# QWERTY6191/projected-lmc

Measured on AMD Instinct MI355X. Metric: MLL+grad iters/sec, n=8192 16-task LMC, higher is better.
Workload: dtype f32; 1 GPU; C3: ProjectedGPModel+ProjectedLMCmll exact training step (PLMC_fast), n=8192 d=8 p=16 q=8 Matern-5/2 fp32; latents sharded q/N per GPU; n_points=8192, n_dim=8, n_tasks=16, n_latents=8, parallelism=latent-shard x1

## Files before the change

### include/plmc.h

```cpp
#ifndef PLMC_H
#define PLMC_H

#include <stddef.h>
#include <stdint.h>

#ifdef __cplusplus
extern "C" {
#endif

enum { PLMC_RBF = 0, PLMC_MATERN12 = 1, PLMC_MATERN32 = 2, PLMC_MATERN52 = 3, PLMC_SPLINE = 4 };

int         plmc_version(void);
int         plmc_block(void);
int64_t     plmc_pad(int64_t n);
int         plmc_max_dim(void);
const char *plmc_last_error(void);
int64_t     plmc_vd_blocks_for(int64_t n_pad, int64_t lda, int elem_bytes);
int64_t     plmc_vd_blocks(int64_t n_pad, int64_t lda);
int64_t     plmc_vd_blocks_keep(int64_t n_pad, int64_t lda);
int64_t     plmc_split_scales_offset(int64_t n_pad, int64_t lda);
int64_t     plmc_grad_scratch_bytes_for(int64_t n_pad, int q, int elem_bytes);
int64_t     plmc_grad_scratch_bytes(int64_t n_pad, int q);
int64_t     plmc_grad_partials_bytes(int64_t n_pad, int q);

// ... 35 lines not shown
int plmc_potrs_aug_f64(double *A, int64_t n_pad, int64_t lda, int naug, int64_t wcol0, int64_t strideA, double *Vd, int q, void *stream);
int plmc_potrs_aug_kept_f32(float *A, int64_t n_pad, int64_t lda, int naug, int64_t wcol0, int64_t strideA, float *Vd, int q,
                            const float *eig_lo, void *stream);
int plmc_potrs_aug_kept_f64(double *A, int64_t n_pad, int64_t lda, int naug, int64_t wcol0, int64_t strideA, double *Vd, int q,
                            const double *eig_lo, void *stream);

int plmc_extract_col_f32(const float *A, int64_t n_pad, int64_t lda, int64_t strideA, int c,
                         float *z, double *quad, int q, void *stream);
int plmc_extract_col_f64(const double *A, int64_t n_pad, int64_t lda, int64_t strideA, int c,
                         double *z, double *quad, int q, void *stream);

int plmc_wt_matvec_f32(const float *W, int64_t n_pad, int64_t ldw, int64_t strideW, const float *z,
                       float *alpha, int q, void *stream);
int plmc_wt_matvec_f64(const double *W, int64_t n_pad, int64_t ldw, int64_t strideW, const double *z,
                       double *alpha, int q, void *stream);

int plmc_trmm_ut_f32(const float *A, int64_t n_pad, int64_t lda, int64_t strideA, int n, const float *Z, int ns, int64_t ldz,
                     int64_t strideZ, const float *shift, float *Y, int64_t ldy, int64_t strideY, int q, void *stream);
int plmc_trmm_ut_f64(const double *A, int64_t n_pad, int64_t lda, int64_t strideA, int n, const double *Z, int ns, int64_t ldz,
                     int64_t strideZ, const double *shift, double *Y, int64_t ldy, int64_t strideY, int q, void *stream);

int plmc_gemm_tn_f32(int mode, int M, int N, int K, const float *A, int64_t lda, int64_t strideA, const float *B,
                     int64_t ldb, int64_t strideB, float *C, int64_t ldc, int64_t strideC, int batch, void *stream);
int plmc_gemm_tn_f64(int mode, int M, int N, int K, const double *A, int64_t lda, int64_t strideA, const double *B,
                     int64_t ldb, int64_t strideB, double *C, int64_t ldc, int64_t strideC, int batch, void *stream);
#define PLMC_TRI_A_LOWER 1
#define PLMC_TRI_B_LOWER 2
#define PLMC_TRI_A_UPPER 4
#define PLMC_TRI_C_LOWER 8
#define PLMC_TRI_C_ZERO 16
// ... 520 lines not shown
```

### projected-lmc_amd/csrc/api.hip

```cpp
#include <stdlib.h>
#include <mutex>
#include <vector>

#include "api_common.hpp"
#include "../../include/plmc.h"

namespace plmc {
char *err_buf() {
  static thread_local char buf[256] = {0};
  return buf;
}

static const char *kProfNames[PK_COUNT] = {"k_assemble", "k_write_rhs", "k_assemble_cross", "k_diag",   "k_panel",
                                           "k_trail",    "k_wdiag",     "k_trtri_row",      "k_extract_col",
                                           "k_wt_matvec", "k_kinv_grad", "k_reduce_grad", "k_kernel_vjp",
                                           "sweep_total", "k_trail_row", "k_trail_head", "k_gpanel", "k_split_w", "k_posterior_moments", "k_trmm_ut",
                                           "k_input_grad", "k_posterior_dx", "k_cross_matvec", "k_cross_matvec_dx"};
struct ProfRec { int id; hipEvent_t a, b; double flops, bytes; };
static unsigned g_prof_mask = 0;
static std::vector<ProfRec> g_recs;
static std::vector<hipEvent_t> g_free;

static hipEvent_t get_event() {
  if (!g_free.empty()) { hipEvent_t e = g_free.back(); g_free.pop_back(); return e; }
// ... 9 lines not shown
static Knobs g_knobs;
static bool g_knobs_loaded = false;
static void load_knobs() {
  const char *h = getenv("PLMC_HALF_TILES"), *g = getenv("PLMC_GRP");
  g_knobs.half_tiles = h ? (atoi(h) == 1 ? 1e30 : (double)atoi(h)) : 640.0;
  g_knobs.grp = g ? atoi(g) : 0;
  g_knobs.serial = getenv("PLMC_SERIAL") && atoi(getenv("PLMC_SERIAL")) != 0;
  g_knobs.bulk_lds = getenv("PLMC_BULK_LDS") ? atoi(getenv("PLMC_BULK_LDS")) : -1;
  g_knobs.split = getenv("PLMC_SPLIT") ? atoi(getenv("PLMC_SPLIT")) : 2;
  if (g_knobs.split != 0 && g_knobs.split != 3) g_knobs.split = 2;
  g_knobs.bulk_streams = getenv("PLMC_BULK_STREAMS") ? atoi(getenv("PLMC_BULK_STREAMS")) : 2;
  g_knobs.chain = getenv("PLMC_CHAIN") ? atoi(getenv("PLMC_CHAIN")) : 1;
  g_knobs.chain_nw = getenv("PLMC_CHAIN_NW") ? atoi(getenv("PLMC_CHAIN_NW")) : 0;
  g_knobs.tail_pair = getenv("PLMC_TAIL_PAIR") ? atoi(getenv("PLMC_TAIL_PAIR")) : 1;
  g_knobs.chain_edge = getenv("PLMC_CHAIN_EDGE") ? atoi(getenv("PLMC_CHAIN_EDGE")) : 0;
  g_knobs_loaded = true;
}
const Knobs &knobs() {
  if (!g_knobs_loaded) {
    std::lock_guard<std::recursive_mutex> lk(g_api_mutex);
    if (!g_knobs_loaded) load_knobs();
  }
  return g_knobs;
}

constexpr int SWEEP_CTX = 2;
struct SweepCtx {
  hipStream_t caller = nullptr;
  bool used = false;
  unsigned long long stamp = 0;
// ... 177 lines not shown
```

### projected-lmc_amd/csrc/api_common.hpp

```cpp
#pragma once
#include <hip/hip_runtime.h>
#include <stdint.h>
#include <stdio.h>
#include <string.h>
#include <type_traits>

#include "gemm_core.hpp"
#include "covariance.hpp"

namespace plmc {

constexpr int MAX_DIM = 32;
constexpr int MAX_COMP = 4;
constexpr int SM_MAX_MIX = 8;
constexpr int SM_MAX_DIM = 8;
constexpr int PER_MAX_DIM = 8;
constexpr int RQ_MAX_DIM = 16;
constexpr int LPER_MAX_DIM = 8;
constexpr int DOT_MAX_DIM = 16;
constexpr int DOT_MAX_POWER = 8;
constexpr int SUM_MAX_DIM = 8;
constexpr int FAM_PUBLIC_BASE = 16;
enum { F_PER = 5, F_RQ = 6, F_LPER = 7 };

// ... 27 lines not shown
  long idx_;
  hipStream_t st_;
};

struct Knobs {
  double half_tiles;
  int grp;
  bool serial;
  int bulk_lds;
  int split;
  int bulk_streams;
  int chain;
  int chain_edge;
  int tail_pair;
  int chain_nw;
};
const Knobs &knobs();

enum CovFamily { COV_PLAIN, COV_ADD, COV_SM, COV_PER, COV_RQ, COV_LPER, COV_SUM, COV_DOT };

constexpr int EVERY_D = 1 << 30, NEVER = 1 << 30;
struct FamilyTraits {
  int max_dim;
  const char *dim_text;
  int max_count;
  const char *count_text;
  bool count_first;
  bool needs_second, needs_third;
  bool rows_per_comp;
  int max_dc;
// ... 142 lines not shown
```

### projected-lmc_amd/csrc/potrf.hip

```cpp
#include <stdlib.h>
#include "api_common.hpp"
#include "covariance.hpp"
#include "diag_block.hpp"
#include "bf3_engine.hpp"
#include "chain_engine.hpp"
#include "vd_layout.hpp"
#include "../../include/plmc.h"

namespace plmc {

template <typename T> constexpr int CHAIN_BURST = sizeof(T) == 8 ? 4 : 8;

template <typename T> struct ColMap {
  int u0, nU, Taug, w0, nW;
  int64_t n_pad;
  T *W;
  int64_t ldw, strideW;
};

template <typename T, int NT, bool BURSTED = false>
__global__ __launch_bounds__(NTHREADS, TILE_MIN_WAVES<T>) void k_panel(T *A, int64_t lda, int64_t strideA, int r, ColMap<T> cm,
                                                     const T *__restrict__ Vd, int64_t strideV) {
  __builtin_amdgcn_s_setprio(3);
  __shared__ __align__(16) T smem[tile_smem_elems<T>()];
// ... 596 lines not shown
    for (int u = 0; u < U; ++u)
#pragma unroll
      for (int e = 0; e < EPV; ++e) s[e] += (double)v[u][e] * (double)zz[u];
  }
#pragma unroll
  for (int e = 0; e < EPV; ++e) red[rg][cl + e] = s[e];
  __syncthreads();
  if (threadIdx.x < CW) {
    double t = 0.0;
#pragma unroll
    for (int g = 0; g < NRG; ++g) t += red[g][threadIdx.x];
    alpha[(int64_t)lat * n_pad + colw + threadIdx.x] = (T)t;
  }
}

template <typename T>
__global__ __launch_bounds__(WTMV_NT) void k_w_diag(const T *__restrict__ W, int64_t n_pad, int64_t ldw, int64_t strideW,
                                                    T *__restrict__ kd) {
  using vec_t = typename Traits<T>::vec_t;
  constexpr int EPV = Traits<T>::EPV;
  constexpr int LPR = 128 / EPV;
  constexpr int NRG = WTMV_NT / LPR;
  __shared__ double red[NRG][NB];
  const int lat = blockIdx.y;
  const int cl = (threadIdx.x % LPR) * EPV, rg = threadIdx.x / LPR;
  const int64_t col0 = (int64_t)blockIdx.x * NB;
  const T *Wl = W + (int64_t)lat * strideW + col0 + cl;
  double s[EPV];
#pragma unroll
  for (int e = 0; e < EPV; ++e) s[e] = 0.0;
// ... 8 lines not shown
    for (int u = 0; u < 4; ++u)
      if (l + u * NRG < n_pad) {
#pragma unroll
        for (int e = 0; e < EPV; ++e) s[e] += (double)v[u][e] * (double)v[u][e];
      }
  }
#pragma unroll
  for (int e = 0; e < EPV; ++e) red[rg][cl + e] = s[e];
  __syncthreads();
  if (threadIdx.x < NB) {
    double t = 0.0;
#pragma unroll
    for (int g = 0; g < NRG; ++g) t += red[g][threadIdx.x];
    kd[(int64_t)lat * n_pad + col0 + threadIdx.x] = (T)t;
  }
}

template <typename T, class S>
struct Sweep {
  static constexpr bool bf3 = !std::is_void<S>::value;
  static_assert(!bf3 || sizeof(T) == 4, "split schemes stand in for fp32 products");
  static constexpr double nb = NB, nb3 = nb * nb * nb, esz = sizeof(T);

  T *A;
  int64_t n_pad, lda, strideA, naug_pad, wcol0;
  int q, m, Taug;
  bool with_inverse, keep;
  const float *eig_lo = nullptr;
  double *logdet = nullptr;
  int *info = nullptr;
  T *Vd, *Wg, *Vg2[2], *Ph, *Pbulk;
  unsigned short *Pl[2], *Praw, *VgP2[2], *Wk, *Uk;
  unsigned short *Pl4 = nullptr;
  float *scl;
  int64_t strideV, pl_lat, sc_lat, uk_step;
  int64_t slot_step = 0;
  bool pair = false;
  T *WA;
  const Knobs &kn;
  double hthr;
  unsigned bulk_lds;
  int grp, ng, chain_pool;
  hipStream_t st, C = nullptr, H = nullptr;
  hipEvent_t e_entry = nullptr, e_v = nullptr, e_gh = nullptr, e_p = nullptr, e_hd = nullptr, e_tail = nullptr, e_doneC = nullptr,
             e_doneH = nullptr, e_prev = nullptr, e_sc = nullptr;

  Sweep(T *A_, int64_t n_pad_, int64_t lda_, int naug, int64_t wcol0_, int64_t strideA_, T *Vd_, int q_, bool with_inverse_, bool keep_,
        int grp_, unsigned bulk_lds_, hipStream_t st_)
      : A(A_), n_pad(n_pad_), lda(lda_), strideA(strideA_), naug_pad(plmc_pad(naug)), wcol0(wcol0_), q(q_), m((int)(n_pad_ / NB)),
        Taug((int)(plmc_pad(naug) / NB)), with_inverse(with_inverse_), keep(keep_), Vd(Vd_), kn(knobs()), hthr(kn.half_tiles),
        bulk_lds(bulk_lds_), grp(grp_), st(st_) {
    const VdLayout L(n_pad, lda, (int)sizeof(T), keep);
    strideV = L.stride();
    pl_lat = L.stride_u16();
    sc_lat = L.stride_f32();
    Wg = L.at<T>(Vd, L.wg);
    Ph = L.at<T>(Vd, L.ph);
// ... 177 lines not shown
      const int nt = cm.nU + cm.Taug + cm.nW;
      if (nt > 0)
        hipLaunchKernelGGL((k_raw_planes<S>), dim3(nt, G0(1), q), dim3(NTHREADS), 0, s, (const float *)A, lda, strideA, 0, cm, Praw, pl_lat, wcol0,
                           (const float *)scl, sc_lat);
    }
  }

  void near(int gi, hipStream_t s) {
    const int g1 = G0(gi + 1), g2 = G0(gi + 2), g3 = G0(gi + 3);
    update(g2, g3 - g2, pair_lo(gi), g1 - 1, cm_buf(g2, m - g2, Taug, 0, g1), s, PK_TRAIL, 0, 0, false, 0, true);
  }
  void far(int gi, hipStream_t s) {
    if (!(gi & 1)) return;
    const int g1 = G0(gi + 1), g3 = G0(gi + 3);
    update(g3, m - g3, pair_lo(gi), g1 - 1, cm_buf(g3, m - g3, Taug, 0, g1), s, PK_TRAIL);
  }

  bool bind_streams() {
    if (!kn.serial) bind_sweep_ctx(st, 8);
    C = kn.serial ? nullptr : side_stream();
    H = kn.serial ? nullptr : (kn.bulk_streams == 1 ? st : side_stream(1));
    hipEvent_t *const ev[] = {&e_entry, &e_v, &e_gh, &e_p, &e_hd, &e_tail, &e_doneC, &e_doneH, &e_prev};
    bool la = C && H && ng > 2;
    for (int i = 0; i < 9; ++i) la = (*ev[i] = sync_event(i)) && la;
    e_sc = sync_event(12);
    return la;
  }

  int inputs(const AssembleJob *job) {
    if (job) {
// ... 18 lines not shown
        gpanel(g0, g1 - g0, cm_buf(g1, g2 - g1, 0, 0, 0), gi & 1, st, 1);
        gpanel(g0, g1 - g0, cm_buf(g2, m - g2, Taug, 0, g0), gi & 1, st, 0);
        if (pair) {
          update(g1, g2 - g1, g0, g1 - 1, cm_buf(g2, m - g2, Taug, 0, g1), st, PK_TRAIL_HEAD, 0, 0, false, g2);
          near(gi, st);
          far(gi, st);
        } else {
          update(g1, m - g1, g0, g1 - 1, cm_buf(g1, m - g1, Taug, 0, g1), st, PK_TRAIL, g2, g2, false, g2);
        }
        update(g1, g2 - g1, g0, g1 - 1, cm_buf(g1, g2 - g1, 0, 0, 0), st, PK_TRAIL_HEAD, 0, 0, true);
      } else {
        gpanel(g0, g1 - g0, cm_buf(g1, m - g1, Taug, 0, g0), gi & 1, st, 0);
        update(g1, m - g1, g0, g1 - 1, cm_buf(g1, m - g1, Taug, 0, g1), st, PK_TRAIL);
      }
    }
    return finish(st);
  }

  int lookahead(const AssembleJob *job) {
    const bool fused = job && e_sc;
    if (fused) {
      const int rc = assemble_rows(*job, (int)sizeof(T), A, lda, strideA, q, 0, G0(1), st, G0(1));
      if (rc != 0) return rc;
      scan(st, 0, (int64_t)G0(1) * NB, 0, SCAN_PARTS / 2);
    } else {
      const int rc = inputs(job);
      if (rc != 0) return rc;
    }
    (void)hipEventRecord(e_entry, st);
    (void)hipStreamWaitEvent(C, e_entry, 0);
// ... 15 lines not shown
      (void)hipEventRecord(e_v, C);
      if (gi > 0 || bf3) (void)hipStreamWaitEvent(C, e_hd, 0);
      gpanel(g0, G, cm_buf(g1, g2 - g1, 0, 0, 0), gi & 1, C, 1);
      (void)hipEventRecord(e_gh, C);
      if (gi > 0) (void)hipStreamWaitEvent(C, e_tail, 0);
      update(g1, g2 - g1, g0, g1 - 1, cm_buf(g1, g2 - g1, 0, 0, 0), C, PK_TRAIL_HEAD, 0, 0, true);

      (void)hipStreamWaitEvent(H, e_v, 0);
      wtri_planes(gi, H);
      gpanel(g0, G, cm_buf(g2, m - g2, Taug, 0, g0), gi & 1, H, 0);
      (void)hipEventRecord(e_p, H);
      (void)hipStreamWaitEvent(H, e_gh, 0);
      if (gi > 0) (void)hipStreamWaitEvent(H, e_tail, 0);
      update(g1, g2 - g1, g0, g1 - 1, cm_buf(g2, m - g2, Taug, 0, g1), H, PK_TRAIL_HEAD, 0, 0, false, g2);
      (void)hipEventRecord(e_hd, H);

      (void)hipStreamWaitEvent(st, e_p, 0);
      (void)hipStreamWaitEvent(st, e_gh, 0);
      if (pair) {
        near(gi, st);
        (void)hipEventRecord(e_tail, st);
        far(gi, st);
      } else {
        update(g2, m - g2, g0, g1 - 1, cm_buf(g2, m - g2, Taug, 0, g1), st, PK_TRAIL);
        (void)hipEventRecord(e_tail, st);
      }
    }
    const int rc_fin = finish(C);
    (void)hipEventRecord(e_doneC, C);
    (void)hipEventRecord(e_doneH, H);
    (void)hipStreamWaitEvent(st, e_doneC, 0);
    (void)hipStreamWaitEvent(st, e_doneH, 0);
    (void)hipEventRecord(e_prev, st);
    return rc_fin;
  }
};

template <typename T, class S>
int potrf_impl(T *A, int64_t n_pad, int64_t lda, int naug, int64_t strideA, T *Vd, double *logdet, int *info,
               int with_inverse_arg, int q, const float *eig_lo, void *stream, const AssembleJob *job = nullptr) {
  PLMC_REQUIRE((with_inverse_arg & 2) == 0, "with_inverse bit 1 (K^-1 accumulated in the sweep) is gone: use plmc_kinv_grad_* behind the sweep");
  const bool with_inverse = (with_inverse_arg & 1) != 0;
  const bool keep = !std::is_void<S>::value && (with_inverse_arg & 4) != 0 && with_inverse;
  PLMC_REQUIRE(A && Vd && logdet && info, "null pointer");
  PLMC_REQUIRE(n_pad > 0 && n_pad % NB == 0 && lda % NB == 0 && lda >= n_pad, "n_pad/lda must be multiples of NB");
  const int64_t naug_pad = plmc_pad(naug);
  PLMC_REQUIRE(naug >= 0 && n_pad + naug_pad + (with_inverse ? n_pad : 0) <= lda,
               "lda too small for naug (+ the n_pad columns of the inverse factor)");
  PLMC_REQUIRE(q > 0 && aligned16(A) && aligned16(Vd), "bad q or unaligned buffer");
  const Knobs &kn = knobs();
  const int grp = (!keep && kn.grp > 0 && kn.grp < GMAX) ? kn.grp : GMAX;
  const unsigned bulk_lds = (unsigned)(kn.bulk_lds >= 0 ? kn.bulk_lds : (q == 1 ? 20000 : (q == 2 ? 16000 : 0)));
  Sweep<T, S> sw(A, n_pad, lda, naug, n_pad + naug_pad, strideA, Vd, q, with_inverse, keep, grp, bulk_lds, (hipStream_t)stream);
  sw.eig_lo = eig_lo;
  sw.logdet = logdet;
  sw.info = info;
  const double npd = (double)n_pad;
  ProfScope whole(PK_SWEEP, sw.st, q * (with_inverse ? 2.0 : 1.0) * npd * npd * npd / 3.0, 0.0);
  sw.clear();
  return sw.bind_streams() ? sw.lookahead(job) : sw.one_stream(job);
}

bool vd_w_planes(const float *Vd, int64_t n_pad, int64_t lda, const unsigned short **wk, int64_t *wk_lat_stride, const float **w_scale,
                 int64_t *w_scale_lat_stride) {
  const VdLayout L(n_pad, lda, 4, false);
  if (L.wk < 0) return false;
  *wk = L.at<const unsigned short>(Vd, L.wk);
  *wk_lat_stride = L.stride_u16();
  *w_scale = L.at<const float>(Vd, L.scl) + SC_SW;
  *w_scale_lat_stride = L.stride_f32();
  return true;
// ... 70 lines not shown
                   void *stream) {
  PLMC_REQUIRE(W && z && alpha, "null pointer");
  PLMC_REQUIRE(q > 0 && n_pad > 0 && n_pad % NB == 0 && ldw >= n_pad, "q > 0, n_pad a positive multiple of NB, ldw >= n_pad");
  PLMC_REQUIRE(aligned16(W) && ldw % Traits<T>::EPV == 0 && strideW % Traits<T>::EPV == 0, "16-byte alignment of W, ldw and strideW");
  ProfScope ps(PK_WTMV, (hipStream_t)stream, q * (double)n_pad * n_pad, q * ((double)n_pad * n_pad / 2) * sizeof(T));
  if ((int64_t)q * (n_pad / NB) < 128)
    hipLaunchKernelGGL((k_wt_matvec<T, 32>), dim3((unsigned)(n_pad / 32), q), dim3(WTMV_NT / 4), 0, (hipStream_t)stream, W, n_pad, ldw, strideW, z,
                       alpha);
  else
    hipLaunchKernelGGL((k_wt_matvec<T, NB>), dim3((unsigned)(n_pad / NB), q), dim3(WTMV_NT), 0, (hipStream_t)stream, W, n_pad, ldw, strideW, z,
                       alpha);
  return launch_status(__func__);
}

template <typename T>
int w_diag_impl(const T *W, int64_t n_pad, int64_t ldw, int64_t strideW, T *kinv_diag, int q, void *stream) {
  PLMC_REQUIRE(W && kinv_diag, "null pointer");
  PLMC_REQUIRE(q > 0 && n_pad > 0 && n_pad % NB == 0 && ldw >= n_pad, "q > 0, n_pad a positive multiple of NB, ldw >= n_pad");
  PLMC_REQUIRE(aligned16(W) && ldw % Traits<T>::EPV == 0 && strideW % Traits<T>::EPV == 0, "16-byte alignment of W, ldw and strideW");
  ProfScope ps(PK_WTMV, (hipStream_t)stream, q * (double)n_pad * n_pad, q * ((double)n_pad * n_pad / 2) * sizeof(T));
  hipLaunchKernelGGL(k_w_diag<T>, dim3((unsigned)(n_pad / NB), q), dim3(WTMV_NT), 0, (hipStream_t)stream, W, n_pad, ldw, strideW,
                     kinv_diag);
  return launch_status(__func__);
}

}

static int potrf_f32_any(float *A, int64_t n_pad, int64_t lda, int naug, int64_t strideA, float *Vd, double *logdet, int *info,
                         int with_inverse, int q, const float *eig_lo, void *stream, const plmc::AssembleJob *job = nullptr) {
  const int split = plmc::knobs().split;
// ... 65 lines not shown
                         int q, void *stream) {
  return plmc::extract_col_impl<float>(A, n_pad, lda, strideA, c, z, quad, q, stream);
}
int plmc_extract_col_f64(const double *A, int64_t n_pad, int64_t lda, int64_t strideA, int c, double *z,
                         double *quad, int q, void *stream) {
  return plmc::extract_col_impl<double>(A, n_pad, lda, strideA, c, z, quad, q, stream);
}
int plmc_wt_matvec_f32(const float *W, int64_t n_pad, int64_t ldw, int64_t strideW, const float *z, float *alpha,
                       int q, void *stream) {
  return plmc::wt_matvec_impl<float>(W, n_pad, ldw, strideW, z, alpha, q, stream);
}
int plmc_wt_matvec_f64(const double *W, int64_t n_pad, int64_t ldw, int64_t strideW, const double *z, double *alpha,
                       int q, void *stream) {
  return plmc::wt_matvec_impl<double>(W, n_pad, ldw, strideW, z, alpha, q, stream);
}
int plmc_w_diag_f32(const float *W, int64_t n_pad, int64_t ldw, int64_t strideW, float *kinv_diag, int q, void *stream) {
  return plmc::w_diag_impl<float>(W, n_pad, ldw, strideW, kinv_diag, q, stream);
}
int plmc_w_diag_f64(const double *W, int64_t n_pad, int64_t ldw, int64_t strideW, double *kinv_diag, int q, void *stream) {
  return plmc::w_diag_impl<double>(W, n_pad, ldw, strideW, kinv_diag, q, stream);
}
}
```

### projected-lmc_amd/projectedlmc/_engine.py

```python
import ctypes
import math
import os

import torch

from . import _hip
from . import settings
from .kernels import dot_power
from ._pivot import PivotCheck, deferred_pivot_checks, walk

LOG2PI = math.log(2.0 * math.pi)


class Workspace:

    def __init__(self, n, q, naug, dtype, device, with_inverse=True, keep_planes=False, ncomp=1, sm=False, per=False):
        L = _hip.lib()
        self.n, self.q, self.naug, self.dtype, self.device = n, q, naug, dtype, device
        self.ncomp = ncomp
        self.with_inverse = bool(with_inverse)
        self.keep_planes = bool(keep_planes) and self.with_inverse and dtype == torch.float32
        self.NB = L.cdll.plmc_block()
        self.n_pad = int(L.cdll.plmc_pad(n))
        self.naug_pad = int(L.cdll.plmc_pad(naug)) if naug > 0 else 0
# ... 4 lines not shown
        self.strideA = self.n_pad * self.lda
        esz = torch.empty((), dtype=dtype).element_size()
        vd_blocks = L.cdll.plmc_vd_blocks_keep(self.n_pad, self.lda) if self.keep_planes else L.cdll.plmc_vd_blocks_for(self.n_pad, self.lda, esz)
        self.Vd = torch.empty(q, int(vd_blocks), self.NB, self.NB, dtype=dtype, device=device)
        self.m = self.n_pad // self.NB
        self.A = torch.empty(q, self.n_pad, self.lda, dtype=dtype, device=device)
        self.logdet = torch.empty(q, dtype=torch.float64, device=device)
        self.quad = torch.empty(q, dtype=torch.float64, device=device)
        self.info = torch.empty(q, dtype=torch.int32, device=device)
        self.z = torch.empty(q, self.n_pad, dtype=dtype, device=device)
        self.W = self.alpha = self.partials = None
        if with_inverse:
            self.W = self.A[:, :, self.wcol0:self.wcol0 + self.n_pad]
            self.ldw, self.strideW = self.lda, self.strideA
            self.alpha = torch.empty(q, self.n_pad, dtype=dtype, device=device)
            nbytes = int(L.cdll.plmc_sm_grad_partials_bytes(self.n_pad, q, ncomp, esz) if sm
                         else L.cdll.plmc_sum_grad_partials_bytes(self.n_pad, q, ncomp, esz) if per == SUM
                         else L.cdll.plmc_lper_grad_partials_bytes(self.n_pad, q, esz) if per == LPER
                         else L.cdll.plmc_per_grad_partials_bytes(self.n_pad, q, esz) if per
                         else L.cdll.plmc_grad_partials_bytes(self.n_pad, q * ncomp))
            self.partials = torch.empty(nbytes // 8, dtype=torch.float64, device=device)


_ws_cache = {}


def _release(ws):
    pending = getattr(ws, "pending", None)
    if pending is not None:
        torch.cuda.current_stream(ws.device).wait_event(pending)
# ... 228 lines not shown
            means.record_stream(stream)
        L.call(_SM[base], dt, *head[1:], ell.shape[2], _hip.ptr(scales), _hip.ptr(means), *tail)
    elif ell.dim() == 3:
        L.call(_ADD[base], dt, *head, ell.shape[1], _hip.ptr(ell), *tail)
    else:
        L.call(base, dt, *head, _hip.ptr(ell), *tail)


def _split_grad_table(g, ell_shape, os_shape):
    ne = 1
    for s_ in ell_shape[1:]:
        ne *= s_
    return g[:, :ne].reshape(ell_shape), g[:, ne], (None if os_shape is None else g[:, ne + 1:].reshape(os_shape))


def factorize(kind, X, ell, oscale, noise, rhs, ws, Xs=None, eig_lo=True):
    L = _hip.lib()
    dt, dev = ws.dtype, ws.device
    st = _hip.stream_ptr(dev)
    k = kind_code(kind)
    q, n, d = ws.q, ws.n, X.shape[1]
    fused = os.environ.get("PLMC_FUSED_ASSEMBLE", "1") != "0"
    if not fused:
        _kernel_call(L, "plmc_assemble", dt, (k, _hip.ptr(X), n, d), ell, (_hip.ptr(oscale), _hip.ptr(noise),
                     _hip.ptr(ws.A), ws.lda, ws.strideA, q, st))
    nrhs = 0 if rhs is None else rhs.shape[1]
    if ws.naug_pad > 0:
        L.call("plmc_write_rhs", dt, _hip.ptr(rhs), nrhs, n, _hip.ptr(ws.A), ws.lda, ws.strideA, 0, ws.naug_pad, q, st)
    if Xs is not None:
        _kernel_call(L, "plmc_assemble_cross", dt, (k, _hip.ptr(X), n, _hip.ptr(Xs), Xs.shape[0], d), ell,
                     (_hip.ptr(oscale), _hip.ptr(ws.A), ws.lda, ws.strideA, ws.n_pad + nrhs, ws.n_pad, q, st))
    flags = (1 | (4 if ws.keep_planes else 0)) if ws.with_inverse else 0
    bound = _hip.ptr(noise) if eig_lo else None
    if fused:
        _kernel_call(L, "plmc_factorize_ex", dt, (k, _hip.ptr(X), n, d), ell, (_hip.ptr(oscale), _hip.ptr(noise), _hip.ptr(ws.A), ws.n_pad,
                     ws.lda, ws.naug, ws.strideA, _hip.ptr(ws.Vd), _hip.ptr(ws.logdet), _hip.ptr(ws.info), flags, q, bound, st))
    else:
        L.call("plmc_potrf_ex", dt, _hip.ptr(ws.A), ws.n_pad, ws.lda, ws.naug, ws.strideA, _hip.ptr(ws.Vd),
               _hip.ptr(ws.logdet), _hip.ptr(ws.info), flags, q, bound, st)


def factorize_checked(kind, X, ell, oscale, noise, rhs, ws, Xs=None, eig_lo=True):
    factorize(kind, X, ell, oscale, noise, rhs, ws, Xs, eig_lo)
    if not settings.check_cholesky.on():
        return 0.0
    check = PivotCheck.eager(ws)
    if not check.failed():
# ... 19 lines not shown
        if dt not in (torch.float32, torch.float64):
            raise TypeError("projectedlmc hot path supports float32 and float64 tensors")
        q, n = y.shape
        d = X.shape[1]
        _check_kernel_shape(L, ell, kind)
        G = n_components(ell, kind)
        need_grad = any(ctx.needs_input_grad[1:5]) or table is not None or x_grad
        Xc, ellc, osc, nzc, yc = (_contig(t, dt) for t in (X, ell, oscale, noise, y))
        ws = get_workspace(n, q, 1, dt, dev, need_grad, G, is_sm(ell), _per_kind(kind))
        st = _hip.stream_ptr(dev)
        grad = table if table is not None else (torch.empty(q, grad_table_width(ell, kind), dtype=torch.float64, device=dev) if need_grad else None)
        check = settings.check_cholesky.on()
        gX = torch.empty(q, n, d, dtype=torch.float64, device=dev) if x_grad else None

        def enqueue(noise_eff):
            factorize(kind, Xc, ellc, osc, noise_eff, yc.reshape(q, 1, n), ws)
            info = PivotCheck(ws) if check else None
            L.call("plmc_extract_col", dt, _hip.ptr(ws.A), ws.n_pad, ws.lda, ws.strideA, 0, _hip.ptr(ws.z),
                   _hip.ptr(ws.quad), q, st)
            if need_grad:
                L.call("plmc_wt_matvec", dt, _hip.ptr(ws.W), ws.n_pad, ws.ldw, ws.strideW, _hip.ptr(ws.z),
                       _hip.ptr(ws.alpha), q, st)
                gs = grad_stream(dev)
                gst = st
                if gs is not None:
                    gs.wait_stream(torch.cuda.current_stream(dev))
                    gst = _hip.stream_handle(gs, dev)
                    for t in (grad, Xc, ellc, osc, noise_eff, gX):
                        if t is not None:
                            t.record_stream(gs)
                Kinv = _kinv_buffer(ws) if x_grad else None
                ldk = Kinv.shape[2] if x_grad else 0
                _kernel_call(L, "plmc_kinv_grad_vd", dt, (kind_code(kind), _hip.ptr(ws.W), ws.n_pad, ws.ldw, ws.strideW,
                             _hip.ptr(ws.alpha), _hip.ptr(Xc), n, d), ellc, (_hip.ptr(osc), _hip.ptr(grad),
                             _hip.ptr(Kinv), ldk, ws.n_pad * ldk, None, _hip.ptr(ws.partials), q, _hip.ptr(noise_eff), _hip.ptr(ws.Vd), gst),
                             stream=gs)
                if x_grad:
# ... 679 lines not shown
```

### projected-lmc_amd/projectedlmc/_hip.py

```python
import ctypes
import os

import torch

_HERE = os.path.dirname(os.path.abspath(__file__))
LIB_PATH = os.environ.get("PLMC_LIB") or os.path.join(_HERE, "libplmc_hip.so")

ABI_VERSION = 4
KIND = {"rbf": 0, "matern12": 1, "matern32": 2, "matern52": 3, "spline": 4}
FAM = {"rbf": 0, "matern12": 1, "matern32": 2, "matern52": 3, "periodic": 16, "rq": 17, "locally_periodic": 18}

_c = ctypes
_P = _c.c_void_p
_I = _c.c_int
_L = _c.c_int64

_TYPED = {
    "plmc_assemble": [_I, _P, _I, _I, _P, _P, _P, _P, _L, _L, _I, _P],
    "plmc_assemble_add": [_I, _P, _I, _I, _I, _P, _P, _P, _P, _L, _L, _I, _P],
    "plmc_assemble_per": [_P, _I, _I, _P, _P, _P, _P, _P, _L, _L, _I, _P],
    "plmc_assemble_lper": [_P, _I, _I, _P, _P, _P, _P, _P, _P, _L, _L, _I, _P],
    "plmc_assemble_sum": [_P, _I, _I, _I, _P, _P, _P, _P, _P, _L, _L, _I, _P],
    "plmc_assemble_rq": [_P, _I, _I, _P, _P, _P, _P, _P, _L, _L, _I, _P],
    "plmc_assemble_dot": [_P, _I, _I, _P, _P, _I, _P, _P, _P, _L, _L, _I, _P],
# ... 9 lines not shown
    "plmc_assemble_cross_sm": [_P, _I, _P, _I, _I, _I, _P, _P, _P, _P, _L, _L, _L, _L, _I, _P],
    "plmc_potrf": [_P, _L, _L, _I, _L, _P, _P, _P, _I, _I, _P],
    "plmc_potrf_ex": [_P, _L, _L, _I, _L, _P, _P, _P, _I, _I, _P, _P],
    "plmc_factorize_ex": [_I, _P, _I, _I, _P, _P, _P, _P, _L, _L, _I, _L, _P, _P, _P, _I, _I, _P, _P],
    "plmc_factorize_add_ex": [_I, _P, _I, _I, _I, _P, _P, _P, _P, _L, _L, _I, _L, _P, _P, _P, _I, _I, _P, _P],
    "plmc_factorize_per_ex": [_P, _I, _I, _P, _P, _P, _P, _P, _L, _L, _I, _L, _P, _P, _P, _I, _I, _P, _P],
    "plmc_factorize_lper_ex": [_P, _I, _I, _P, _P, _P, _P, _P, _P, _L, _L, _I, _L, _P, _P, _P, _I, _I, _P, _P],
    "plmc_factorize_sum_ex": [_P, _I, _I, _I, _P, _P, _P, _P, _P, _L, _L, _I, _L, _P, _P, _P, _I, _I, _P, _P],
    "plmc_factorize_rq_ex": [_P, _I, _I, _P, _P, _P, _P, _P, _L, _L, _I, _L, _P, _P, _P, _I, _I, _P, _P],
    "plmc_factorize_dot_ex": [_P, _I, _I, _P, _P, _I, _P, _P, _P, _L, _L, _I, _L, _P, _P, _P, _I, _I, _P, _P],
    "plmc_factorize_sm_ex": [_P, _I, _I, _I, _P, _P, _P, _P, _P, _L, _L, _I, _L, _P, _P, _P, _I, _I, _P, _P],
    "plmc_potrs_aug": [_P, _L, _L, _I, _L, _L, _P, _I, _P],
    "plmc_potrs_aug_kept": [_P, _L, _L, _I, _L, _L, _P, _I, _P, _P],
    "plmc_extract_col": [_P, _L, _L, _L, _I, _P, _P, _I, _P],
    "plmc_wt_matvec": [_P, _L, _L, _L, _P, _P, _I, _P],
    "plmc_w_diag": [_P, _L, _L, _L, _P, _I, _P],
    "plmc_trmm_ut": [_P, _L, _L, _L, _I, _P, _I, _L, _L, _P, _P, _L, _L, _I, _P],
    "plmc_gemm_tn": [_I, _I, _I, _I, _P, _L, _L, _P, _L, _L, _P, _L, _L, _I, _P],
    "plmc_gemm_tn_tri": [_I, _I, _I, _I, _I, _P, _L, _L, _P, _L, _L, _P, _L, _L, _I, _P],
    "plmc_kinv_grad": [_I, _P, _L, _L, _L, _P, _P, _I, _I, _P, _P, _P, _P, _L, _L, _P, _P, _I, _P],
    "plmc_kinv_grad_ex": [_I, _P, _L, _L, _L, _P, _P, _I, _I, _P, _P, _P, _P, _L, _L, _P, _P, _I, _P, _P],
    "plmc_kinv_grad_vd": [_I, _P, _L, _L, _L, _P, _P, _I, _I, _P, _P, _P, _P, _L, _L, _P, _P, _I, _P, _P, _P],
    "plmc_kinv_grad_add_vd": [_I, _P, _L, _L, _L, _P, _P, _I, _I, _I, _P, _P, _P, _P, _L, _L, _P, _P, _I, _P, _P, _P],
    "plmc_kinv_grad_per_vd": [_P, _L, _L, _L, _P, _P, _I, _I, _P, _P, _P, _P, _P, _L, _L, _P, _P, _I, _P, _P, _P],
    "plmc_kinv_grad_lper_vd": [_P, _L, _L, _L, _P, _P, _I, _I, _P, _P, _P, _P, _P, _P, _L, _L, _P, _P, _I, _P, _P, _P],
    "plmc_kinv_grad_sum_vd": [_P, _L, _L, _L, _P, _P, _I, _I, _I, _P, _P, _P, _P, _P, _L, _L, _P, _P, _I, _P, _P, _P],
    "plmc_kinv_grad_rq_vd": [_P, _L, _L, _L, _P, _P, _I, _I, _P, _P, _P, _P, _P, _L, _L, _P, _P, _I, _P, _P, _P],
    "plmc_kinv_grad_dot_vd": [_P, _L, _L, _L, _P, _P, _I, _I, _P, _P, _I, _P, _P, _P, _L, _L, _P, _P, _I, _P, _P, _P],
    "plmc_kinv_grad_sm_vd": [_P, _L, _L, _L, _P, _P, _I, _I, _I, _P, _P, _P, _P, _P, _L, _L, _P, _P, _I, _P, _P, _P],
    "plmc_loo_grad": [_I, _P, _L, _L, _L, _L, _P, _P, _I, _I, _P, _P, _P, _P, _I, _P],
# ... 45 lines not shown
    "plmc_kernel_vjp": [_I, _P, _I, _P, _I, _I, _P, _P, _P, _L, _L, _P, _P, _P, _I, _P],
    "plmc_kernel_vjp_add": [_I, _P, _I, _P, _I, _I, _I, _P, _P, _P, _L, _L, _P, _P, _P, _I, _P],
    "plmc_qr_small": [_P, _I, _I, _L, _P, _L, _P, _L, _P],
    "plmc_comm_allreduce_sum": [_P, _L, _P],
    "plmc_posterior_moments": [_P, _L, _L, _L, _I, _P, _P, _I, _P],
    "plmc_mix_posterior": [_P, _P, _P, _I, _I, _I, _c.c_double, _P, _P, _P],
}
_PLAIN = {
    "plmc_version": ([], _I),
    "plmc_block": ([], _I),
    "plmc_pad": ([_L], _L),
    "plmc_vd_blocks": ([_L, _L], _L),
    "plmc_vd_blocks_for": ([_L, _L, _I], _L),
    "plmc_vd_blocks_keep": ([_L, _L], _L),
    "plmc_split_scales_offset": ([_L, _L], _L),
    "plmc_max_dim": ([], _I),
    "plmc_max_components": ([], _I),
    "plmc_sm_max_mixtures": ([], _I),
    "plmc_sm_max_dim": ([], _I),
    "plmc_sm_grad_partials_bytes": ([_L, _I, _I, _I], _L),
    "plmc_per_max_dim": ([], _I),
    "plmc_per_grad_partials_bytes": ([_L, _I, _I], _L),
    "plmc_lper_max_dim": ([], _I),
    "plmc_lper_grad_partials_bytes": ([_L, _I, _I], _L),
    "plmc_sum_max_components": ([], _I),
    "plmc_sum_max_dim": ([], _I),
    "plmc_sum_grad_partials_bytes": ([_L, _I, _I, _I], _L),
    "plmc_rq_max_dim": ([], _I),
    "plmc_dot_max_dim": ([], _I),
    "plmc_dot_max_power": ([], _I),
# ... 158 lines not shown
```

Measured before the change: 60.77 iters/sec.

## Overlap W^T z matvec with Cholesky sweep via per-group partial accumulation

Splits the alpha = W^T z matvec into row-range partial sums that are launched on the head stream as each group of the inverse factor finishes, accumulating into a float64 buffer. A final kernel adds the last group's rows, writes alpha, and also extracts z and the quadratic term, replacing the separate extract_col and wt_matvec launches. The goal is to hide the matvec inside the factorization sweep and remove a full serial pass over W after it. The cost is extra launches, an fp64 accumulator buffer, and reliance on thread-local arming state shared between the Python and C layers.

Result: no change. 61.30 iters/sec, median of 6 (+0.9%).

```diff
diff --git a/include/plmc.h b/include/plmc.h
--- a/include/plmc.h
+++ b/include/plmc.h
@@ -73,6 +73,10 @@
                        float *alpha, int q, void *stream);
 int plmc_wt_matvec_f64(const double *W, int64_t n_pad, int64_t ldw, int64_t strideW, const double *z,
                        double *alpha, int q, void *stream);
+
+int plmc_alpha_partials_arm_f32(float *z, double *quad, float *alpha, double *acc, int c, void *stream);
+int plmc_alpha_partials_arm_f64(double *z, double *quad, double *alpha, double *acc, int c, void *stream);
+int plmc_alpha_partials_ranges(int64_t n_pad, int grp, int64_t *r0r1, int cap);
 
 int plmc_trmm_ut_f32(const float *A, int64_t n_pad, int64_t lda, int64_t strideA, int n, const float *Z, int ns, int64_t ldz,
                      int64_t strideZ, const float *shift, float *Y, int64_t ldy, int64_t strideY, int q, void *stream);
diff --git a/projected-lmc_amd/csrc/api.hip b/projected-lmc_amd/csrc/api.hip
--- a/projected-lmc_amd/csrc/api.hip
+++ b/projected-lmc_amd/csrc/api.hip
@@ -47,6 +47,7 @@
   g_knobs.chain_nw = getenv("PLMC_CHAIN_NW") ? atoi(getenv("PLMC_CHAIN_NW")) : 0;
   g_knobs.tail_pair = getenv("PLMC_TAIL_PAIR") ? atoi(getenv("PLMC_TAIL_PAIR")) : 1;
   g_knobs.chain_edge = getenv("PLMC_CHAIN_EDGE") ? atoi(getenv("PLMC_CHAIN_EDGE")) : 0;
+  g_knobs.alpha_partials = getenv("PLMC_ALPHA_PARTIALS") ? atoi(getenv("PLMC_ALPHA_PARTIALS")) : 1;
   g_knobs_loaded = true;
 }
 const Knobs &knobs() {
diff --git a/projected-lmc_amd/csrc/api_common.hpp b/projected-lmc_amd/csrc/api_common.hpp
--- a/projected-lmc_amd/csrc/api_common.hpp
+++ b/projected-lmc_amd/csrc/api_common.hpp
@@ -65,6 +65,7 @@
   int chain_edge;
   int tail_pair;
   int chain_nw;
+  int alpha_partials;
 };
 const Knobs &knobs();
 
diff --git a/projected-lmc_amd/csrc/potrf.hip b/projected-lmc_amd/csrc/potrf.hip
--- a/projected-lmc_amd/csrc/potrf.hip
+++ b/projected-lmc_amd/csrc/potrf.hip
@@ -634,6 +634,107 @@
   }
 }
 
+constexpr int AWT_NT = 256, AWT_U = 8;
+template <typename T, int CW>
+__device__ __forceinline__ void awt_strip(const T *__restrict__ Wl, int64_t ldw, const T *__restrict__ zc, int64_t lda, int64_t l0, int64_t l1,
+                                          double *red) {
+  using vec_t = typename Traits<T>::vec_t;
+  constexpr int EPV = Traits<T>::EPV, LPR = CW / EPV, NRG = AWT_NT / LPR;
+  const int cl = (threadIdx.x % LPR) * EPV, rg = threadIdx.x / LPR;
+  double s[EPV];
+#pragma unroll
+  for (int e = 0; e < EPV; ++e) s[e] = 0.0;
+  for (int64_t l = l0 + rg; l < l1; l += AWT_U * NRG) {
+    vec_t v[AWT_U];
+    T zz[AWT_U];
+#pragma unroll
+    for (int u = 0; u < AWT_U; ++u) {
+      const int64_t ll = l + u * NRG;
+      const int64_t lc = ll < l1 ? ll : l1 - 1;
+      v[u] = *reinterpret_cast<const vec_t *>(Wl + lc * ldw + cl);
+      const T zv = zc[lc * lda];
+      zz[u] = ll < l1 ? zv : T(0);
+    }
+#pragma unroll
+    for (int u = 0; u < AWT_U; ++u)
+#pragma unroll
+      for (int e = 0; e < EPV; ++e) s[e] += (double)v[u][e] * (double)zz[u];
+  }
+#pragma unroll
+  for (int e = 0; e < EPV; ++e) red[rg * CW + cl + e] = s[e];
+}
+template <typename T, int CW>
+__device__ __forceinline__ double awt_total(const double *red) {
+  constexpr int NRG = AWT_NT / (CW / Traits<T>::EPV);
+  double t = 0.0;
+#pragma unroll
+  for (int g = 0; g < NRG; ++g) t += red[g * CW + threadIdx.x];
+  return t;
+}
+
+template <typename T, int CW>
+__global__ __launch_bounds__(AWT_NT, 2) void k_wt_matvec_rows(const T *__restrict__ W, int64_t ldw, int64_t strideW, const T *__restrict__ zcol,
+                                                              int64_t lda, int64_t strideA, int64_t r0, int64_t r1, double *acc, int64_t n_pad) {
+  __shared__ double red[AWT_NT * Traits<T>::EPV];
+  const int lat = blockIdx.y;
+  const int64_t colw = (int64_t)blockIdx.x * CW;
+  const int64_t col0 = colw / NB * NB;
+  awt_strip<T, CW>(W + (int64_t)lat * strideW + colw, ldw, zcol + (int64_t)lat * strideA, lda, col0 > r0 ? col0 : r0, r1, red);
+  __syncthreads();
+  if (threadIdx.x < CW) {
+    const double t = awt_total<T, CW>(red);
+    double *a = acc + (int64_t)lat * n_pad + colw + threadIdx.x;
+    *a = col0 >= r0 ? t : *a + t;
+  }
+}
+
+template <typename T, int CW>
+__global__ __launch_bounds__(AWT_NT, 2) void k_alpha_finish(const T *__restrict__ W, int64_t ldw, int64_t strideW, const T *__restrict__ zcol,
+                                                            int64_t lda, int64_t strideA, int64_t r0, const double *__restrict__ acc, int64_t n_pad,
+                                                            T *__restrict__ alpha, T *__restrict__ z, double *__restrict__ quad) {
+  static_assert(AWT_NT == NTHREADS, "quad is summed in k_extract_col's order");
+  __shared__ double red[AWT_NT * Traits<T>::EPV];
+  const int lat = blockIdx.y;
+  const T *zc = zcol + (int64_t)lat * strideA;
+  if (blockIdx.x == 0) {
+    double *rq = red;
+    double s = 0.0;
+    for (int64_t i0 = threadIdx.x; i0 < n_pad; i0 += (int64_t)AWT_U * NTHREADS) {
+      T v[AWT_U];
+#pragma unroll
+      for (int u = 0; u < AWT_U; ++u) {
+        const int64_t i = i0 + (int64_t)u * NTHREADS;
+        v[u] = zc[(i < n_pad ? i : n_pad - 1) * lda];
+      }
+#pragma unroll
+      for (int u = 0; u < AWT_U; ++u) {
+        const int64_t i = i0 + (int64_t)u * NTHREADS;
+        if (i < n_pad) {
+          z[(int64_t)lat * n_pad + i] = v[u];
+          s += (double)v[u] * (double)v[u];
+        }
+      }
+    }
+    rq[threadIdx.x] = s;
+    __syncthreads();
+    for (int o = NTHREADS / 2; o > 0; o >>= 1) {
+      if (threadIdx.x < o) rq[threadIdx.x] += rq[threadIdx.x + o];
+      __syncthreads();
+    }
+    if (threadIdx.x == 0) quad[lat] = rq[0];
+    return;
+  }
+  const int64_t colw = (int64_t)(blockIdx.x - 1) * CW;
+  const int64_t col0 = colw / NB * NB;
+  awt_strip<T, CW>(W + (int64_t)lat * strideW + colw, ldw, zc, lda, col0 > r0 ? col0 : r0, n_pad, red);
+  __syncthreads();
+  if (threadIdx.x < CW) {
+    const double t = awt_total<T, CW>(red);
+    const int64_t c = (int64_t)lat * n_pad + colw + threadIdx.x;
+    alpha[c] = (T)(col0 >= r0 ? t : acc[c] + t);
+  }
+}
+
 template <typename T>
 __global__ __launch_bounds__(WTMV_NT) void k_w_diag(const T *__restrict__ W, int64_t n_pad, int64_t ldw, int64_t strideW,
                                                     T *__restrict__ kd) {
@@ -672,6 +773,21 @@
     for (int g = 0; g < NRG; ++g) t += red[g][threadIdx.x];
     kd[(int64_t)lat * n_pad + col0 + threadIdx.x] = (T)t;
   }
+}
+
+struct AlphaJob {
+  void *z, *alpha;
+  double *quad, *acc;
+  int c;
+};
+static thread_local AlphaJob t_alpha_job;
+static thread_local void *t_alpha_stream = nullptr;
+static thread_local int t_alpha_elem = 0;
+inline int alpha_groups(int m, int grp) { return (m + grp - 1) / grp; }
+inline void alpha_range(int m, int grp, int gi, int64_t *r0, int64_t *r1) {
+  const int g0 = gi * grp < m ? gi * grp : m, g1 = (gi + 1) * grp < m ? (gi + 1) * grp : m;
+  *r0 = (int64_t)g0 * NB;
+  *r1 = (int64_t)g1 * NB;
 }
 
 template <typename T, class S>
@@ -699,6 +815,7 @@
   double hthr;
   unsigned bulk_lds;
   int grp, ng, chain_pool;
+  const AlphaJob *aj = nullptr;
   hipStream_t st, C = nullptr, H = nullptr;
   hipEvent_t e_entry = nullptr, e_v = nullptr, e_gh = nullptr, e_p = nullptr, e_hd = nullptr, e_tail = nullptr, e_doneC = nullptr,
              e_doneH = nullptr, e_prev = nullptr, e_sc = nullptr;
@@ -906,6 +1023,31 @@
     if (!(gi & 1)) return;
     const int g1 = G0(gi + 1), g3 = G0(gi + 3);
     update(g3, m - g3, pair_lo(gi), g1 - 1, cm_buf(g3, m - g3, Taug, 0, g1), s, PK_TRAIL);
+  }
+
+  void alpha_rows(int gi, hipStream_t s) {
+    if (!aj || gi + 1 >= ng) return;
+    int64_t r0, r1;
+    alpha_range(m, grp, gi, &r0, &r1);
+    ProfScope ps(PK_WTMV, s, q * 2.0 * (double)(r1 - r0) * (r0 + r1) / 2, q * (double)(r1 - r0) * (r0 + r1) / 2 * esz);
+    if (kn.alpha_partials == 2)
+      hipLaunchKernelGGL((k_wt_matvec_rows<T, 32>), dim3((unsigned)(r1 / 32), q), dim3(AWT_NT), 0, s, (const T *)WA, lda, strideA,
+                         (const T *)(A + n_pad + aj->c), lda, strideA, r0, r1, aj->acc, n_pad);
+    else
+      hipLaunchKernelGGL((k_wt_matvec_rows<T, NB>), dim3((unsigned)(r1 / NB), q), dim3(AWT_NT), 0, s, (const T *)WA, lda, strideA,
+                         (const T *)(A + n_pad + aj->c), lda, strideA, r0, r1, aj->acc, n_pad);
+  }
+  void alpha_finish(hipStream_t s) {
+    if (!aj) return;
+    int64_t r0, r1;
+    alpha_range(m, grp, ng - 1, &r0, &r1);
+    ProfScope ps(PK_WTMV, s, q * 2.0 * (double)(r1 - r0) * (r0 + r1) / 2, q * ((double)(r1 - r0) * (r0 + r1) / 2 + 2.0 * n_pad) * esz);
+    if (kn.alpha_partials == 2)
+      hipLaunchKernelGGL((k_alpha_finish<T, 32>), dim3((unsigned)(1 + n_pad / 32), q), dim3(AWT_NT), 0, s, (const T *)WA, lda, strideA,
+                         (const T *)(A + n_pad + aj->c), lda, strideA, r0, (const double *)aj->acc, n_pad, (T *)aj->alpha, (T *)aj->z, aj->quad);
+    else
+      hipLaunchKernelGGL((k_alpha_finish<T, NB>), dim3((unsigned)(1 + n_pad / NB), q), dim3(AWT_NT), 0, s, (const T *)WA, lda, strideA,
+                         (const T *)(A + n_pad + aj->c), lda, strideA, r0, (const double *)aj->acc, n_pad, (T *)aj->alpha, (T *)aj->z, aj->quad);
   }
 
   bool bind_streams() {
@@ -954,6 +1096,8 @@
         update(g1, m - g1, g0, g1 - 1, cm_buf(g1, m - g1, Taug, 0, g1), st, PK_TRAIL);
       }
     }
+    for (int gi = 0; gi + 1 < ng; ++gi) alpha_rows(gi, st);
+    alpha_finish(st);
     return finish(st);
   }
 
@@ -999,6 +1143,7 @@
       if (gi > 0) (void)hipStreamWaitEvent(H, e_tail, 0);
       update(g1, g2 - g1, g0, g1 - 1, cm_buf(g2, m - g2, Taug, 0, g1), H, PK_TRAIL_HEAD, 0, 0, false, g2);
       (void)hipEventRecord(e_hd, H);
+      alpha_rows(gi, H);
 
       (void)hipStreamWaitEvent(st, e_p, 0);
       (void)hipStreamWaitEvent(st, e_gh, 0);
@@ -1012,6 +1157,7 @@
       }
     }
     const int rc_fin = finish(C);
+    alpha_finish(H);
     (void)hipEventRecord(e_doneC, C);
     (void)hipEventRecord(e_doneH, H);
     (void)hipStreamWaitEvent(st, e_doneC, 0);
@@ -1040,6 +1186,15 @@
   sw.eig_lo = eig_lo;
   sw.logdet = logdet;
   sw.info = info;
+  AlphaJob alpha_job;
+  if (with_inverse_arg & 8) {
+    const bool armed = t_alpha_elem == (int)sizeof(T) && t_alpha_stream == stream;
+    t_alpha_elem = 0;
+    PLMC_REQUIRE(armed, "with_inverse bit 3 needs plmc_alpha_partials_arm_* of this element type on this stream right before the call");
+    PLMC_REQUIRE(with_inverse && t_alpha_job.c < naug, "with_inverse bit 3 needs the inverse factor and a live augmented column");
+    alpha_job = t_alpha_job;
+    sw.aj = &alpha_job;
+  }
   const double npd = (double)n_pad;
   ProfScope whole(PK_SWEEP, sw.st, q * (with_inverse ? 2.0 : 1.0) * npd * npd * npd / 3.0, 0.0);
   sw.clear();
@@ -1140,6 +1295,18 @@
 }
 
 template <typename T>
+int alpha_arm_impl(T *z, double *quad, T *alpha, double *acc, int c, void *stream) {
+  t_alpha_elem = 0;
+  if (!knobs().alpha_partials) return 0;
+  PLMC_REQUIRE(z && quad && alpha && acc, "null pointer");
+  PLMC_REQUIRE(c >= 0, "column outside the augmented block");
+  t_alpha_job = AlphaJob{z, alpha, quad, acc, c};
+  t_alpha_stream = stream;
+  t_alpha_elem = (int)sizeof(T);
+  return 1;
+}
+
+template <typename T>
 int w_diag_impl(const T *W, int64_t n_pad, int64_t ldw, int64_t strideW, T *kinv_diag, int q, void *stream) {
   PLMC_REQUIRE(W && kinv_diag, "null pointer");
   PLMC_REQUIRE(q > 0 && n_pad > 0 && n_pad % NB == 0 && ldw >= n_pad, "q > 0, n_pad a positive multiple of NB, ldw >= n_pad");
@@ -1235,6 +1402,22 @@
                        int q, void *stream) {
   return plmc::wt_matvec_impl<double>(W, n_pad, ldw, strideW, z, alpha, q, stream);
 }
+int plmc_alpha_partials_arm_f32(float *z, double *quad, float *alpha, double *acc, int c, void *stream) {
+  return plmc::alpha_arm_impl<float>(z, quad, alpha, acc, c, stream);
+}
+int plmc_alpha_partials_arm_f64(double *z, double *quad, double *alpha, double *acc, int c, void *stream) {
+  return plmc::alpha_arm_impl<double>(z, quad, alpha, acc, c, stream);
+}
+int plmc_alpha_partials_ranges(int64_t n_pad, int grp, int64_t *r0r1, int cap) {
+  PLMC_REQUIRE(n_pad > 0 && n_pad % plmc::NB == 0 && r0r1, "n_pad must be a positive multiple of plmc_block(), r0r1 not null");
+  const int kg = plmc::knobs().grp;
+  if (grp <= 0) grp = kg;
+  if (grp <= 0 || grp > plmc::GMAX) grp = plmc::GMAX;
+  const int m = (int)(n_pad / plmc::NB), ng = plmc::alpha_groups(m, grp);
+  PLMC_REQUIRE(cap >= ng, "r0r1 holds fewer than (n_pad / plmc_block() + grp - 1) / grp pairs");
+  for (int gi = 0; gi < ng; ++gi) plmc::alpha_range(m, grp, gi, r0r1 + 2 * gi, r0r1 + 2 * gi + 1);
+  return ng;
+}
 int plmc_w_diag_f32(const float *W, int64_t n_pad, int64_t ldw, int64_t strideW, float *kinv_diag, int q, void *stream) {
   return plmc::w_diag_impl<float>(W, n_pad, ldw, strideW, kinv_diag, q, stream);
 }
diff --git a/projected-lmc_amd/projectedlmc/_engine.py b/projected-lmc_amd/projectedlmc/_engine.py
--- a/projected-lmc_amd/projectedlmc/_engine.py
+++ b/projected-lmc_amd/projectedlmc/_engine.py
@@ -42,6 +42,7 @@
             self.W = self.A[:, :, self.wcol0:self.wcol0 + self.n_pad]
             self.ldw, self.strideW = self.lda, self.strideA
             self.alpha = torch.empty(q, self.n_pad, dtype=dtype, device=device)
+            self.alpha_acc = torch.empty(q, self.n_pad, dtype=torch.float64, device=device)
             nbytes = int(L.cdll.plmc_sm_grad_partials_bytes(self.n_pad, q, ncomp, esz) if sm
                          else L.cdll.plmc_sum_grad_partials_bytes(self.n_pad, q, ncomp, esz) if per == SUM
                          else L.cdll.plmc_lper_grad_partials_bytes(self.n_pad, q, esz) if per == LPER
@@ -300,7 +301,16 @@
     return g[:, :ne].reshape(ell_shape), g[:, ne], (None if os_shape is None else g[:, ne + 1:].reshape(os_shape))
 
 
-def factorize(kind, X, ell, oscale, noise, rhs, ws, Xs=None, eig_lo=True):
+def arm_alpha(ws, st):
+    L = _hip.lib()
+    fn = getattr(L.cdll, "plmc_alpha_partials_arm" + ("_f32" if ws.dtype == torch.float32 else "_f64"))
+    rc = fn(_hip.ptr(ws.z), _hip.ptr(ws.quad), _hip.ptr(ws.alpha), _hip.ptr(ws.alpha_acc), 0, st)
+    if rc < 0:
+        raise RuntimeError("plmc_alpha_partials_arm failed (%d): %s" % (rc, L.cdll.plmc_last_error().decode()))
+    return rc == 1
+
+
+def factorize(kind, X, ell, oscale, noise, rhs, ws, Xs=None, eig_lo=True, alpha=False):
     L = _hip.lib()
     dt, dev = ws.dtype, ws.device
     st = _hip.stream_ptr(dev)
@@ -316,7 +326,7 @@
     if Xs is not None:
         _kernel_call(L, "plmc_assemble_cross", dt, (k, _hip.ptr(X), n, _hip.ptr(Xs), Xs.shape[0], d), ell,
                      (_hip.ptr(oscale), _hip.ptr(ws.A), ws.lda, ws.strideA, ws.n_pad + nrhs, ws.n_pad, q, st))
-    flags = (1 | (4 if ws.keep_planes else 0)) if ws.with_inverse else 0
+    flags = (1 | (4 if ws.keep_planes else 0) | (8 if alpha else 0)) if ws.with_inverse else 0
     bound = _hip.ptr(noise) if eig_lo else None
     if fused:
         _kernel_call(L, "plmc_factorize_ex", dt, (k, _hip.ptr(X), n, d), ell, (_hip.ptr(oscale), _hip.ptr(noise), _hip.ptr(ws.A), ws.n_pad,
@@ -366,13 +376,16 @@
         gX = torch.empty(q, n, d, dtype=torch.float64, device=dev) if x_grad else None
 
         def enqueue(noise_eff):
-            factorize(kind, Xc, ellc, osc, noise_eff, yc.reshape(q, 1, n), ws)
+            partials = need_grad and arm_alpha(ws, st)
+            factorize(kind, Xc, ellc, osc, noise_eff, yc.reshape(q, 1, n), ws, alpha=partials)
             info = PivotCheck(ws) if check else None
-            L.call("plmc_extract_col", dt, _hip.ptr(ws.A), ws.n_pad, ws.lda, ws.strideA, 0, _hip.ptr(ws.z),
-                   _hip.ptr(ws.quad), q, st)
+            if not partials:
+                L.call("plmc_extract_col", dt, _hip.ptr(ws.A), ws.n_pad, ws.lda, ws.strideA, 0, _hip.ptr(ws.z),
+                       _hip.ptr(ws.quad), q, st)
             if need_grad:
-                L.call("plmc_wt_matvec", dt, _hip.ptr(ws.W), ws.n_pad, ws.ldw, ws.strideW, _hip.ptr(ws.z),
-                       _hip.ptr(ws.alpha), q, st)
+                if not partials:
+                    L.call("plmc_wt_matvec", dt, _hip.ptr(ws.W), ws.n_pad, ws.ldw, ws.strideW, _hip.ptr(ws.z),
+                           _hip.ptr(ws.alpha), q, st)
                 gs = grad_stream(dev)
                 gst = st
                 if gs is not None:
diff --git a/projected-lmc_amd/projectedlmc/_hip.py b/projected-lmc_amd/projectedlmc/_hip.py
--- a/projected-lmc_amd/projectedlmc/_hip.py
+++ b/projected-lmc_amd/projectedlmc/_hip.py
@@ -47,6 +47,7 @@
     "plmc_potrs_aug_kept": [_P, _L, _L, _I, _L, _L, _P, _I, _P, _P],
     "plmc_extract_col": [_P, _L, _L, _L, _I, _P, _P, _I, _P],
     "plmc_wt_matvec": [_P, _L, _L, _L, _P, _P, _I, _P],
+    "plmc_alpha_partials_arm": [_P, _P, _P, _P, _I, _P],
     "plmc_w_diag": [_P, _L, _L, _L, _P, _I, _P],
     "plmc_trmm_ut": [_P, _L, _L, _L, _I, _P, _I, _L, _L, _P, _P, _L, _L, _I, _P],
     "plmc_gemm_tn": [_I, _I, _I, _I, _P, _L, _L, _P, _L, _L, _P, _L, _L, _I, _P],
@@ -122,6 +123,7 @@
     "plmc_vd_blocks_for": ([_L, _L, _I], _L),
     "plmc_vd_blocks_keep": ([_L, _L], _L),
     "plmc_split_scales_offset": ([_L, _L], _L),
+    "plmc_alpha_partials_ranges": ([_L, _I, _P, _I], _I),
     "plmc_max_dim": ([], _I),
     "plmc_max_components": ([], _I),
     "plmc_sm_max_mixtures": ([], _I),
```
